# Wenlin-Chen/ADKF-IFT

Measured on AMD Instinct MI355X. Metric: meta-tasks/sec (N_support=128, d=256), higher is better.
Workload: dtype f32

## Files before the change

### adkf_ift_amd/csrc/adkf_gp.hip

```cpp
#include <hip/hip_runtime.h>
#include <algorithm>
#include <cstdio>
#include <cstdlib>

#include "../../include/adkf_gp.h"
#include "ard.h"
#include "pna.h"
#include "readout.h"
#include "block.h"
#include "outer_step.h"
#include "refine64.h"
#include "hyper.h"
#include "large_fused.h"
#include "gemm_x3.h"
#include "dense_x3.h"
#include "dist_task.h"
#include "dz_task.h"
#include "predict_stream.h"
#include "thompson_stream.h"
#include "believer_stream.h"
#include "mes_stream.h"
#include "gumbel_stream.h"
#include "gibbon_stream.h"
#include "kg_stream.h"
#include "jes_stream.h"
#include "ipv_stream.h"
#include "jackknife_stream.h"
#include "ehvi_stream.h"
#include "mix_stream.h"

#include "host_common.h"
#include "host_gp.h"
#include "host_ard.h"
#include "host_stream.h"

extern "C" {

const char* adkf_last_hip_error(void) { return hipGetErrorString(g_last_hip_error); }

const char* adkf_version(void) { return "adkf_gp 0.1 (gfx950)"; }

int adkf_path_info(int32_t ns_max, int32_t nq_max) {
    if (ns_max <= 0 || nq_max < 0 || ns_max > MAX_POINTS || nq_max > MAX_POINTS) return ADKF_E_SIZE;
    int bits = 0;
    const int hi = ns_max > nq_max ? ns_max : nq_max;
    if (nq_max > 0 && use_fused_outer(ns_max, nq_max)) bits |= ADKF_PATH_FUSED_OUTER;
    if (hi > REG_POINTS) { bits |= ADKF_PATH_BLOCKED; if (lg_fused_by_size(hi)) bits |= ADKF_PATH_BLOCKED_FUSED; }
    if (carve(nullptr, 1, ns_max, nq_max > 0 ? nq_max : 1, 4).w64_stride != 0) bits |= ADKF_PATH_R64_REGION;
    if (refine64_lds_optin()) bits |= ADKF_PATH_R64_LDS;
    return bits;
}

int adkf_max_points(void) { return MAX_POINTS; }

size_t adkf_workspace_bytes(int32_t T, int32_t ns_max, int32_t nq_max, int32_t d) {
    if (T <= 0 || ns_max <= 0 || nq_max < 0 || d <= 0) return 0;
    return carve(nullptr, T, ns_max, nq_max, d).bytes;
}

size_t adkf_workspace_bytes_ard(int32_t T, int32_t ns_max, int32_t nq_max, int32_t d) {
    if (T <= 0 || ns_max <= 0 || nq_max < 0 || d <= 0) return 0;
    return carve_ard(nullptr, carve(nullptr, T, ns_max, nq_max, d).bytes, T, ns_max, nq_max, d).bytes;
}

static int median_core(const adkf_batch_t* b, const Workspace& w, float* l0, const InitArgs& init, bool* fused, hipStream_t st) {
    int rc = stage_dist(b, w, has_query(b), st);
    if (rc) return rc;
    *fused = b->ns_max <= 256;
    if (b->ns_max <= 128) k_median<512, 16><<<grid_for(b->T, 1), 512, 0, st>>>(w.D2ss, b->n_s, b->ns_max, l0, b->T, init);
    else if (b->ns_max <= 256) k_median<1024, 32><<<grid_for(b->T, 1), 1024, 0, st>>>(w.D2ss, b->n_s, b->ns_max, l0, b->T, init);
    else {
        LgMedian lm{w.D2ss, b->n_s, b->ns_max, l0, b->T, reinterpret_cast<uint32_t*>(w.lg_med), w.lg_med + b->T, w.lg_med + 2 * (size_t)b->T};
        hipMemsetAsync(lm.hist, 0, sizeof(int) * 256 * (size_t)b->T, st);
        const int rows_blocks = ceil_div(b->ns_max, 16) < 64 ? ceil_div(b->ns_max, 16) : 64;
        for (int pass = 0; pass < 4; ++pass) {
            k_lg_med_hist<<<dim3(rows_blocks, b->T), 256, 0, st>>>(lm, pass);
            k_lg_med_pick<<<ceil_div(b->T, 64), 64, 0, st>>>(lm, pass);
        }
    }
    LAUNCH_OK();
    return 0;
}

int adkf_median_lengthscale(const adkf_batch_t* b, float* l0, void* ws, size_t ws_bytes, void* stream) {
    int rc = check_batch(b, false);
    if (rc) return rc;
    if (!l0 || !ws) return ADKF_E_BADARG;
    Workspace w = carve_for(b, ws);
    if (ws_bytes < w.bytes) return ADKF_E_WORKSPACE;
    bool fused;
    return median_core(b, w, l0, InitArgs{0, 0, nullptr, nullptr}, &fused, static_cast<hipStream_t>(stream));
}

int adkf_init_params(const adkf_batch_t* b, int32_t use_numeric_labels, int32_t use_lengthscale_prior, float* phi,
                     float* priors, float* l0, void* ws, size_t ws_bytes, void* stream) {
    int rc = check_batch(b, false);
    if (rc) return rc;
    if (!phi || !priors || !ws) return ADKF_E_BADARG;
    Workspace w = carve_for(b, ws);
    if (ws_bytes < w.bytes) return ADKF_E_WORKSPACE;
    float* l0p = l0 ? l0 : w.l0;
    hipStream_t st = static_cast<hipStream_t>(stream);
    InitArgs init{use_numeric_labels, use_lengthscale_prior, phi, priors};
    ArdWs a{};
    if (is_ard(b)) {
        a = carve_ard(ws, w.bytes, b->T, b->ns_max, b->nq_max, b->d);
        if (ws_bytes < a.bytes) return ADKF_E_WORKSPACE;
        init.phi = a.phi3;
    }
    bool fused = false;
    rc = median_core(b, w, l0p, init, &fused, st);
    if (rc) return rc;
    if (!fused) k_init_params<<<ceil_div(b->T, 64), 64, 0, st>>>(l0p, b->T, init);
    if (is_ard(b)) k_ard_expand_phi<<<dim3(ceil_div(2 + b->d, 256), b->T), 256, 0, st>>>(a.phi3, phi, b->T, 2 + b->d);
    LAUNCH_OK();
    return 0;
}

int adkf_mll_value_grad(const adkf_batch_t* b, const float* phi, float* f_in, float* g_phi, float* dZ_s, int32_t* info,
                        void* ws, size_t ws_bytes, void* stream) {
    int rc = check_batch(b, false);
    if (rc) return rc;
    if (!phi || !f_in || !info || !ws || !b->y_s || !b->priors) return ADKF_E_BADARG;
    if (is_ard(b)) {
        ArdCtx c;
        adkf_batch_t b0 = *b; b0.flags &= ~ADKF_BATCH_REUSE_INNER;
        rc = ard_setup(&b0, ws, ws_bytes, static_cast<hipStream_t>(stream), c);
        if (rc) return rc;
        rc = ard_eval(c, phi, f_in, g_phi ? g_phi : c.a.ge, info);
        if (rc) return rc;
        if (dZ_s) {
            ArdDzFin fs{c.v, c.a.G, nullptr, nullptr, nullptr, 0.f, dZ_s, b->n_s, c.ns};
            k_ard_dz_fin<<<dim3(ceil_div(c.d, 256), c.ns, c.T), 256, 0, c.st>>>(fs);
            LAUNCH_OK();
        }
        return 0;
    }
    Workspace w = carve_for(b, ws);
    if (ws_bytes < w.bytes) return ADKF_E_WORKSPACE;
    hipStream_t st = static_cast<hipStream_t>(stream);
    rc = stage_dist(b, w, has_query(b), st);
    if (rc) return rc;
    InnerArgs ia = inner_args(b, w, const_cast<float*>(phi), info);
    ia.f_out = f_in; ia.g_out = g_phi;
    rc = launch_inner(ia, w, st);
    if (rc) return rc;
    launch_refine(make_tv(b, w, false), b, w, false, 0, nullptr, info, st, f_in, g_phi, nullptr);
    if (dZ_s) {
        TaskView tv = make_tv(b, w, false);
        const int win_tiles = std::max(1, std::min(64, b->ns_max * b->ns_max / 2048));
        WinArgs wa{tv, w.Ainv, w.D2ss, w.Wss, w.scal, b->T, win_tiles};
// ... 295 lines not shown
```

### adkf_ift_amd/csrc/dist_task.h

```cpp
#pragma once
#include "kernels.h"
#include "gemm_x3.h"

namespace adkf {

constexpr int DT_N = 128, DT_NT = 512, DT_PLANE = DT_N * X3_RS, DT_OPER = 3 * DT_PLANE, DT_BUF = 2 * DT_OPER;
constexpr int DT_LDS_BYTES = 2 * DT_BUF * (int)sizeof(unsigned short);

struct DistTaskArgs {
    const float *Zs, *Zq, *mean;
    float *D2ss, *D2qs, *D2qq;
    int d, T;
};

extern __shared__ __attribute__((aligned(16))) unsigned short dt_lds[];

__global__ __launch_bounds__(DT_NT) void k_dist_task(DistTaskArgs a) {
    constexpr int MI = 4, MJ = 2, IH = 1;
    int t, tile;
    if (!task_tile(a.T, 1, t, tile)) return;
    __shared__ float rowsq[2][DT_N];
    const int tid = threadIdx.x, lane = tid & 63, wv = tid >> 6;
    const int wr = wv >> 2, wc = (wv & 3) ^ (wr << 1), fi = lane & 15, fk = lane >> 4;
    const int d = a.d, nc = d / GK, last = nc - 1;
    const bool sym_on = !(wr == 1 && wc < 2);

    const int sr = tid >> 3, sk = (tid & 7) * 4;
    const char* const zs = reinterpret_cast<const char*>(a.Zs + (size_t)t * DT_N * d);
    const char* const zq = reinterpret_cast<const char*>(a.Zq + (size_t)t * DT_N * d);
    const char* const mu = reinterpret_cast<const char*>(a.mean + (size_t)t * d);
    const size_t hi = (size_t)256 * d;
    const uint32_t off = 4u * (uint32_t)(sr * d + sk), off_mu = 4u * (uint32_t)sk;
    auto ldb = [](const char* base, uint32_t o) __attribute__((always_inline)) { return *reinterpret_cast<const float4*>(base + o); };
    const int frag_a = (wr * 64 + fi) * X3_RS + 8 * fk, frag_b = (wc * 32 + fi) * X3_RS + 8 * fk;

    float4 rs[2][2], rq[2][2], rm;
    float sqs[2] = {0.f, 0.f}, sqq[2] = {0.f, 0.f};
    auto fetch = [&](auto with_s, int set, int c) __attribute__((always_inline)) {
        const size_t k = (size_t)(4 * GK) * c;
        if constexpr (decltype(with_s)::value) { rs[set][0] = ldb(zs + k, off); rs[set][1] = ldb(zs + hi + k, off); }
        rq[set][0] = ldb(zq + k, off); rq[set][1] = ldb(zq + hi + k, off);
    };
    auto fetch_mean = [&](int c) __attribute__((always_inline)) { rm = ldb(mu + (size_t)(4 * GK) * c, off_mu); };
    auto centre = [](const float4& r, const float4& m, float (&v)[4]) __attribute__((always_inline)) {
        constexpr int DPP_IDENTITY = 0xE4;
        v[0] = dpp_f<DPP_IDENTITY>(r.x) - m.x; v[1] = dpp_f<DPP_IDENTITY>(r.y) - m.y;
        v[2] = dpp_f<DPP_IDENTITY>(r.z) - m.z; v[3] = dpp_f<DPP_IDENTITY>(r.w) - m.w;
    };
    auto stage = [&](auto with_s, int buf, int set, bool commit) __attribute__((always_inline)) {
        constexpr bool S = decltype(with_s)::value;
        unsigned short* B = dt_lds + buf * DT_BUF;
        float v[2][4], ts[2] = {sqs[0], sqs[1]}, tq[2] = {sqq[0], sqq[1]};
        if constexpr (S) {
            centre(rs[set][0], rm, v[0]); centre(rs[set][1], rm, v[1]);
            x3_stage<true, DT_N, DT_NT, 1>(B, v, ts);
        }
        centre(rq[set][0], rm, v[0]); centre(rq[set][1], rm, v[1]);
        x3_stage<true, DT_N, DT_NT, S ? 1 : 0>(B + DT_OPER, v, tq);
        if constexpr (S) {
#pragma unroll
            for (int ps = 0; ps < 2; ++ps) { sqs[ps] = commit ? ts[ps] : sqs[ps]; sqq[ps] = commit ? tq[ps] : sqq[ps]; }
        }
    };

    auto block_terms = [&](const unsigned short* Ab, const unsigned short* Bb, const bf16x8 (&b)[2][MJ], f32x4 (&acc)[MI][MJ], f32x4 (&small)[MI][MJ]) __attribute__((always_inline)) {
#define ADKF_DT_LOADA(dst_, q_) _Pragma("unroll") for (int i = 0; i < IH; ++i) dst_[i] = *reinterpret_cast<const bf16x8*>(Ab + (q_) * DT_PLANE + (ih + i) * 16 * X3_RS);
#define ADKF_DT_TERM(dst_, av_, bq_)                                                                       \
    _Pragma("unroll") for (int i = 0; i < IH; ++i) _Pragma("unroll") for (int j = 0; j < MJ; ++j)        \
        dst_[ih + i][j] = __builtin_amdgcn_mfma_f32_16x16x32_bf16(bq_[j], av_[i], dst_[ih + i][j], 0, 0, 0);
#pragma unroll
        for (int ih = 0; ih < MI; ih += IH) {
            bf16x8 a0[IH], ax[IH], b2[MJ];
#pragma unroll
            for (int j = 0; j < MJ; ++j) b2[j] = *reinterpret_cast<const bf16x8*>(Bb + 2 * DT_PLANE + j * 16 * X3_RS);
            ADKF_DT_LOADA(a0, 0) ADKF_DT_TERM(small, a0, b2)
            ADKF_DT_LOADA(ax, 2) ADKF_DT_TERM(small, ax, b[0])
            ADKF_DT_LOADA(ax, 1) ADKF_DT_TERM(small, ax, b[1])
            ADKF_DT_TERM(acc, a0, b[0])
            ADKF_DT_TERM(small, a0, b[1]) ADKF_DT_TERM(small, ax, b[0])
        }
#undef ADKF_DT_TERM
#undef ADKF_DT_LOADA
    };
    auto load_b = [&](const unsigned short* Bb, bf16x8 (&b)[2][MJ]) __attribute__((always_inline)) {
#pragma unroll
        for (int q = 0; q < 2; ++q)
#pragma unroll
            for (int j = 0; j < MJ; ++j) b[q][j] = *reinterpret_cast<const bf16x8*>(Bb + q * DT_PLANE + j * 16 * X3_RS);
    };
    auto run_pass = [&](auto with_s, auto&& multiply) __attribute__((always_inline)) {
        auto advance = [&](int c, int nbuf, int nset, bool commit) __attribute__((always_inline)) {
            stage(with_s, nbuf, nset, commit);
            fetch_mean(min(c + 2, last));
            __builtin_amdgcn_sched_barrier(0);
            fetch(with_s, nset, min(c + 3, last));
        };
        stage(with_s, 0, 0, true);
        fetch_mean(min(1, last));
        __builtin_amdgcn_sched_barrier(0);
        fetch(with_s, 0, min(2, last));
        __syncthreads();
        int c = 0;
        for (; c + 1 < nc; c += 2) {
            multiply(0); advance(c, 1, 1, true); __syncthreads();
            multiply(1); advance(c + 1, 0, 0, c + 2 < nc); __syncthreads();
        }
        if (c < nc) { multiply(0); __syncthreads(); }
    };
    auto zero = [](f32x4 (&x)[MI][MJ]) __attribute__((always_inline)) {
#pragma unroll
        for (int i = 0; i < MI; ++i)
#pragma unroll
            for (int j = 0; j < MJ; ++j) x[i][j] = (f32x4){0.f, 0.f, 0.f, 0.f};
    };
    auto values = [&](const f32x4& acc, const float* nrow, const float* ncol, int gi, int gj0, float (&v)[4]) __attribute__((always_inline)) {
        const float nx = nrow[gi];
        const float4 ny = *reinterpret_cast<const float4*>(ncol + gj0);
        v[0] = fmaxf(nx + ny.x - 2.f * acc[0], 0.f); v[1] = fmaxf(nx + ny.y - 2.f * acc[1], 0.f);
        v[2] = fmaxf(nx + ny.z - 2.f * acc[2], 0.f); v[3] = fmaxf(nx + ny.w - 2.f * acc[3], 0.f);
    };
    auto store_sym = [&](float* D, const f32x4& acc, const float* nrm, int rt, int ct) __attribute__((always_inline)) {
        const int gi = rt * 16 + fi, gj0 = ct * 16 + fk * 4;
        float v[4];
        values(acc, nrm, nrm, gi, gj0, v);
        if (rt < ct) {
            *reinterpret_cast<float4*>(D + (size_t)gi * DT_N + gj0) = make_float4(v[0], v[1], v[2], v[3]);
#pragma unroll
            for (int r = 0; r < 4; ++r) D[(size_t)(gj0 + r) * DT_N + gi] = v[r];
        } else {
#pragma unroll
            for (int r = 0; r < 4; ++r) {
                const int gj = gj0 + r;
                if (gi == gj) D[(size_t)gi * DT_N + gj] = 0.f;
                else if (gi < gj) { D[(size_t)gi * DT_N + gj] = v[r]; D[(size_t)gj * DT_N + gi] = v[r]; }
            }
        }
    };

    const std::true_type pass1{};
    const std::false_type pass2{};
    float* const Dss = a.D2ss + (size_t)t * DT_N * DT_N;
    float* const Dqs = a.D2qs + (size_t)t * DT_N * DT_N;
    float* const Dqq = a.D2qq + (size_t)t * DT_N * DT_N;

    fetch_mean(0);
    __builtin_amdgcn_sched_barrier(0);
    fetch(pass1, 0, 0); fetch(pass1, 1, min(1, last));
    {
        f32x4 acc_s[MI][MJ], small_s[MI][MJ], acc_q[MI][MJ], small_q[MI][MJ];
        zero(acc_s); zero(small_s); zero(acc_q); zero(small_q);
        run_pass(pass1, [&](int buf) __attribute__((always_inline)) {
            const unsigned short* S = dt_lds + buf * DT_BUF;
            bf16x8 b[2][MJ];
            load_b(S + frag_b, b);
            if (sym_on) block_terms(S + frag_a, S + frag_b, b, acc_s, small_s);
            __builtin_amdgcn_sched_barrier(0);
            block_terms(S + DT_OPER + frag_a, S + frag_b, b, acc_q, small_q);
        });
        fetch_mean(0);
        __builtin_amdgcn_sched_barrier(0);
        fetch(pass2, 0, 0); fetch(pass2, 1, min(1, last));
#pragma unroll
        for (int ps = 0; ps < 2; ++ps) {
            float s = sqs[ps], q = sqq[ps];
            s += dpp_f<DPP_XOR1>(s); s += dpp_f<DPP_XOR2>(s); s += dpp_f<DPP_HALF_MIRROR>(s);
            q += dpp_f<DPP_XOR1>(q); q += dpp_f<DPP_XOR2>(q); q += dpp_f<DPP_HALF_MIRROR>(q);
            if ((tid & 7) == 0) { rowsq[0][sr + ps * 64] = s; rowsq[1][sr + ps * 64] = q; }
        }
        __syncthreads();
#pragma unroll
        for (int i = 0; i < MI; ++i)
#pragma unroll
            for (int j = 0; j < MJ; ++j) {
                const int rt = wr * 4 + i, ct = wc * 2 + j;
                float v[4];
                values(acc_q[i][j] + small_q[i][j], rowsq[1], rowsq[0], rt * 16 + fi, ct * 16 + fk * 4, v);
                *reinterpret_cast<float4*>(Dqs + (size_t)(rt * 16 + fi) * DT_N + ct * 16 + fk * 4) = make_float4(v[0], v[1], v[2], v[3]);
                if (rt <= ct) store_sym(Dss, acc_s[i][j] + small_s[i][j], rowsq[0], rt, ct);
            }
    }

    {
        f32x4 acc_g[MI][MJ], small_g[MI][MJ];
        zero(acc_g); zero(small_g);
        run_pass(pass2, [&](int buf) __attribute__((always_inline)) {
            if (sym_on) {
                const unsigned short* Q = dt_lds + buf * DT_BUF + DT_OPER;
                bf16x8 b[2][MJ];
                load_b(Q + frag_b, b);
                block_terms(Q + frag_a, Q + frag_b, b, acc_g, small_g);
            }
        });
#pragma unroll
        for (int i = 0; i < MI; ++i)
#pragma unroll
            for (int j = 0; j < MJ; ++j) {
                const int rt = wr * 4 + i, ct = wc * 2 + j;
                if (rt <= ct) store_sym(Dqq, acc_g[i][j] + small_g[i][j], rowsq[1], rt, ct);
            }
    }
}

}
```

### adkf_ift_amd/csrc/host_gp.h

```cpp
#pragma once
#include "host_common.h"

namespace {

inline bool x3_for(int d) { return d >= GK; }

struct Workspace {
    float *mean, *D2ss, *D2qs, *D2qq, *Ainv, *P, *C, *S, *OC, *Wss, *Wqs, *Wqq, *vecs, *scal, *part_oc, *part_ma, *l0;
    float *lg_Dinv, *lg_C, *lg_F, *lg_logdet, *lg_part, *lg_pext;
    int32_t *lg_info, *lg_med, *lg_cnt;
    FitShared* lg_fit;
    double* w64; size_t w64_stride;
    int vld, nt_oc, nt_ma;
    int lg_mode;
    size_t bytes;
};

Workspace carve(void* base, int T, int ns, int nq, int d) {
    Workspace w{};
    Arena ar{static_cast<char*>(base), 0};
    const size_t Tz = (size_t)T;
    w.vld = ns > nq ? ns : nq;
    w.nt_oc = nq > 0 ? tiles_of(nq, ns) : 0;
    w.nt_ma = tiles_of(ns, ns);
    w.mean = ar.floats(Tz * d);
    w.D2ss = ar.floats(Tz * ns * ns);
    w.D2qs = ar.floats(Tz * nq * ns);
    w.D2qq = ar.floats(Tz * nq * nq);
    w.Ainv = ar.floats(Tz * ns * ns);
    w.P = ar.floats(Tz * ns * ns);
    w.C = ar.floats(Tz * nq * ns);
    w.S = ar.floats(Tz * nq * nq);
    w.OC = ar.floats(Tz * nq * ns);
    w.Wss = ar.floats(Tz * ns * ns);
    w.Wqs = ar.floats(Tz * nq * ns);
    w.Wqq = ar.floats(Tz * nq * nq);
    w.vecs = ar.floats(Tz * NVEC * w.vld);
    w.scal = ar.floats(Tz * NSCAL);
    w.part_oc = ar.floats(Tz * (w.nt_oc > 0 ? w.nt_oc : 1) * 4);
    w.part_ma = ar.floats(Tz * w.nt_ma * 4);
    w.l0 = ar.floats(Tz);
    if (w.vld > REG_POINTS) {
        w.lg_Dinv = ar.floats(2 * Tz * LB * LB);
        w.lg_C = ar.floats(Tz * LB * w.vld);
        w.lg_F = ar.floats(Tz * LB * w.vld);
        w.lg_logdet = ar.floats(Tz);
        w.lg_pext = ar.floats(Tz * 2);
        const size_t tq = (size_t)((nq + GT - 1) / GT) * ((nq + GT - 1) / GT);
        const size_t ts = (size_t)((ns + GT - 1) / GT) * ((ns + GT - 1) / GT);
        w.lg_part = ar.floats(Tz * (ts > tq ? ts : tq) * 8);
        w.lg_info = ar.as<int32_t>(Tz);
        w.lg_cnt = ar.as<int32_t>(Tz);
        w.lg_med = ar.as<int32_t>(Tz * 258);
        static_assert(sizeof(FitShared) % sizeof(float) == 0, "FitShared is carved as whole floats");
        w.lg_fit = ar.as<FitShared>(Tz);
    }
    if (w.vld <= r64_maxn()) {
        w.w64_stride = refine64_doubles(ns, nq);
        w.w64 = ar.as<double>(Tz * w.w64_stride);
    }
    w.bytes = ar.off;
    return w;
}

Workspace carve_for(const adkf_batch_t* b, void* ws) {
    Workspace w = carve(ws, b->T, b->ns_max, b->nq_max, b->d);
    w.lg_mode = (b->flags & ADKF_BATCH_LG_UNFUSED) ? -1 : (b->flags & ADKF_BATCH_LG_FUSED) ? 1 : 0;
    return w;
}

int check_batch(const adkf_batch_t* b, bool need_query) {
    (void)hipGetLastError();
    if (!b || b->T <= 0 || b->ns_max <= 0 || b->d <= 0 || !b->Z_s) return ADKF_E_BADARG;
    if (b->kernel != ADKF_KERNEL_RBF && b->kernel != ADKF_KERNEL_MATERN52) return ADKF_E_BADARG;
    if (b->ns_max > MAX_POINTS) return ADKF_E_SIZE;
    if (need_query) {
        if (b->nq_max <= 0 || !b->Z_q) return ADKF_E_BADARG;
        if (b->nq_max > MAX_POINTS) return ADKF_E_SIZE;
    }
    return 0;
}

bool vec_ok(const adkf_batch_t* b, const Workspace& w) {
    if ((b->ns_max & 3) || (b->nq_max & 3) || (b->d & 3) || (w.vld & 3)) return false;
    return aligned16(b->Z_s) && aligned16(b->Z_q) && aligned16(w.mean);
}

TaskView make_tv(const adkf_batch_t* b, const Workspace& w, bool with_query) {
    TaskView tv;
    tv.n_s = b->n_s; tv.n_q = with_query ? b->n_q : nullptr;
    tv.ns_ld = b->ns_max; tv.nq_ld = with_query ? b->nq_max : 0; tv.vld = w.vld; tv.kind = b->kernel;
    tv.scal = w.scal; tv.vecs = w.vecs;
    tv.vec = vec_ok(b, w);
    return tv;
}

inline bool has_query(const adkf_batch_t* b) { return b->nq_max > 0 && b->Z_q != nullptr; }
inline bool is_ard(const adkf_batch_t* b) { return (b->flags & ADKF_BATCH_ARD) != 0; }

bool use_dist_task(const adkf_batch_t* b, const Workspace& w, bool with_query, int parts) {
    static const bool optin = lds_optin(DT_LDS_BYTES, {kernel_ptr(&k_dist_task)});
    return optin && parts == 3 && with_query && b->ns_max == DT_N && b->nq_max == DT_N && !b->n_s && !b->n_q && (b->d % GK) == 0 &&
           b->d <= (1 << 22) && vec_ok(b, w);
}

int stage_dist(const adkf_batch_t* b, const Workspace& w, bool with_query, hipStream_t st, int parts = 3) {
    if (b->flags & ADKF_BATCH_REUSE_DIST) return 0;
    const int T = b->T, ns = b->ns_max, nq = with_query ? b->nq_max : 0, d = b->d;
    if (!(parts & 2)) with_query = false;
    if ((parts & 1) && !(parts & 4)) k_colmean<<<dim3(ceil_div(d, 64), T), 256, 0, st>>>(b->Z_s, b->n_s, ns, d, w.mean, T);
    if (use_dist_task(b, w, with_query, parts)) {
        k_dist_task<<<grid_for(T, 1), DT_NT, DT_LDS_BYTES, st>>>(DistTaskArgs{b->Z_s, b->Z_q, w.mean, w.D2ss, w.D2qs, w.D2qq, d, T});
        LAUNCH_OK();
        return 0;
    }
    ProbDist p;
    p.mean = w.mean; p.d = d; p.vec = vec_ok(b, w);
    ProbDistMulti pm;
    pm.vec = p.vec; pm.end0 = pm.end1 = 0; pm.tn0 = pm.tn1 = pm.tn2 = 1;
    int nblk = 0, total = 0;
    auto add = [&](const ProbDist& q, int M, int N) {
        const int tn = ceil_div(N, GT), tiles = ceil_div(M, GT) * tn;
        if (nblk == 0) { pm.s0 = q; pm.tn0 = tn; pm.end0 = pm.end1 = total + tiles; pm.s1 = pm.s2 = q; }
        else if (nblk == 1) { pm.s1 = q; pm.tn1 = tn; pm.end1 = total + tiles; pm.s2 = q; }
        else { pm.s2 = q; pm.tn2 = tn; }
        total += tiles; ++nblk;
    };
    if (parts & 1) {
        p.X = b->Z_s; p.Y = b->Z_s; p.n_x = b->n_s; p.n_y = b->n_s; p.x_ld = ns; p.y_ld = ns; p.symmetric = true; p.D2 = w.D2ss;
        add(p, ns, ns);
    }
    if (with_query) {
        p.X = b->Z_q; p.Y = b->Z_s; p.n_x = b->n_q; p.n_y = b->n_s; p.x_ld = nq; p.y_ld = ns; p.symmetric = false; p.D2 = w.D2qs;
        add(p, nq, ns);
        p.X = b->Z_q; p.Y = b->Z_q; p.n_x = b->n_q; p.n_y = b->n_q; p.x_ld = nq; p.y_ld = nq; p.symmetric = true; p.D2 = w.D2qq;
        add(p, nq, nq);
    }
    if (nblk > 0) {
        if (x3_for(d)) k_bgemm3<ProbDistMulti, GT, 256><<<grid_for(T, total), 256, 0, st>>>(pm, T, 1, total);
        else k_bgemm<ProbDistMulti, GT><<<grid_for(T, total), 256, 0, st>>>(pm, T, 1, total);
    }
    LAUNCH_OK();
    return 0;
}

template <int NMAX, int NT, bool LOW>
void launch_inner_kl(const InnerArgs& a, hipStream_t st) {
    constexpr size_t cache_bytes = sizeof(float) * NMAX * NMAX;
    static const bool optin = lds_optin(cache_bytes, {kernel_ptr(&k_inner<NMAX, NT, 0, LOW>), kernel_ptr(&k_inner<NMAX, NT, 1, LOW>)});
    (void)optin;
    if (a.kind == ADKF_KERNEL_RBF) k_inner<NMAX, NT, 0, LOW><<<grid_for(a.T, 1), NT, cache_bytes, st>>>(a);
    else k_inner<NMAX, NT, 1, LOW><<<grid_for(a.T, 1), NT, cache_bytes, st>>>(a);
}

template <int NMAX, int NT>
void launch_inner_k(const InnerArgs& a, hipStream_t st) {
    if constexpr (NMAX == 128) {
        if (a.T > num_cus()) { launch_inner_kl<NMAX, NT, true>(a, st); return; }
    }
    launch_inner_kl<NMAX, NT, false>(a, st);
}

inline bool lg_fused_by_size(int ld) { return ld >= 4 * LB; }

LgMat lg_mat(const Workspace& w, float* M, int ld, const int32_t* n_arr, const FitShared* fit, int T) {
    LgMat m;
    m.M = M; m.ld = ld; m.n_arr = n_arr; m.fit = fit;
    m.Dinv = w.lg_Dinv; m.Cbuf = w.lg_C; m.Fbuf = w.lg_F; m.logdet = w.lg_logdet; m.pext = w.lg_pext; m.info = w.lg_info;
    const bool fused = w.lg_mode > 0 || (w.lg_mode == 0 && lg_fused_by_size(ld));
    m.cnt = fused ? w.lg_cnt : nullptr;
    m.T = T; m.vec = (ld & 3) == 0;
    return m;
}

void lg_sweep(const LgMat& m0, hipStream_t st) {
    const int nb = ceil_div(m0.ld, LB), tn = ceil_div(m0.ld, GT);
    LgMat m = m0;
    if (m.cnt) {
        float* dinv[2] = {m0.Dinv, m0.Dinv + (size_t)m0.T * LB * LB};
        const int npair = lgf_npair(tn);
        k_lg_diag<<<grid_for(m.T, 1), 512, 0, st>>>(m, 0);
        for (int step = 0; step < nb; ++step) {
            m.Dinv = dinv[step & 1];
            ProbLgPanel pp; pp.m = m; pp.step = step;
            k_bgemm<ProbLgPanel><<<grid_for(m.T, 2 * tn), 256, 0, st>>>(pp, m.T, 2, tn);
            LgStepArgs sa{m, dinv[(step + 1) & 1], m.cnt, step, tn, npair, step + 1 < nb ? 1 : 0};
            k_lg_update_sweep<<<grid_for(m.T, npair), LGF_NT, 0, st>>>(sa);
        }
        return;
    }
    for (int step = 0; step < nb; ++step) {
        k_lg_diag<<<grid_for(m.T, 1), 512, 0, st>>>(m, step);
        ProbLgPanel pp; pp.m = m; pp.step = step;
        k_bgemm<ProbLgPanel><<<grid_for(m.T, 2 * tn), 256, 0, st>>>(pp, m.T, 2, tn);
        ProbLgUpdate pu; pu.m = m; pu.step = step; pu.tri = tn * (tn + 1) / 2;
        k_bgemm<ProbLgUpdate><<<grid_for(m.T, pu.tri), 256, 0, st>>>(pu, m.T, tn, tn);
// ... 265 lines not shown
```

### adkf_ift_amd/csrc/kernels.h

```cpp
#pragma once
#include "problems.h"
#include "inner.h"

namespace adkf {

__global__ __launch_bounds__(256) void k_colmean(const float* Zs, const int32_t* n_s, int ns_ld, int d, float* mean, int T) {
    __shared__ float part[16][64];
    const int t = blockIdx.y;
    const int n = n_s ? n_s[t] : ns_ld;
    const float* Z = Zs + (size_t)t * ns_ld * d;
    const bool vec = (d & 3) == 0 && (reinterpret_cast<uintptr_t>(Zs) & 15) == 0;
    if (vec) {
        const int q = threadIdx.x & 15, g = threadIdx.x >> 4, c4 = blockIdx.x * 64 + q * 4;
        float4 s = make_float4(0.f, 0.f, 0.f, 0.f);
        if (c4 < d) {
            for (int i0 = g; i0 < n; i0 += 16 * 8) {
                float4 v[8];
#pragma unroll
                for (int u = 0; u < 8; ++u) {
                    const int i = i0 + 16 * u;
                    v[u] = *reinterpret_cast<const float4*>(Z + (size_t)(i < n ? i : n - 1) * d + c4);
                }
#pragma unroll
                for (int u = 0; u < 8; ++u)
                    if (i0 + 16 * u < n) { s.x += v[u].x; s.y += v[u].y; s.z += v[u].z; s.w += v[u].w; }
            }
        }
        *reinterpret_cast<float4*>(&part[g][q * 4]) = s;
        __syncthreads();
        const int cl = threadIdx.x, c = blockIdx.x * 64 + cl;
        if (cl < 64 && c < d) {
            float r = 0.f;
#pragma unroll
            for (int k = 0; k < 16; ++k) r += part[k][cl];
            mean[(size_t)t * d + c] = n > 0 ? r / (float)n : 0.f;
        }
        return;
    }
    const int cl = threadIdx.x & 63, g = threadIdx.x >> 6;
    const int c = blockIdx.x * 64 + cl;
    float s = 0.f;
    if (c < d)
        for (int i = g; i < n; i += 4) s += Z[(size_t)i * d + c];
    part[g][cl] = s;
    __syncthreads();
    if (g == 0 && c < d) {
        s = (part[0][cl] + part[1][cl]) + (part[2][cl] + part[3][cl]);
        mean[(size_t)t * d + c] = n > 0 ? s / (float)n : 0.f;
    }
}

struct ProbDist {
    static constexpr bool A_KCONTIG = true, B_KCONTIG = true;
    static constexpr int NRED = 0;
    const float *X, *Y, *mean; const int32_t *n_x, *n_y; int x_ld, y_ld, d; bool symmetric; float* D2;
    int mx, my, i_base, j_base; const float *Xi, *Yi, *mu, *nxi, *nyi; float* Do; bool vec;
    __device__ bool setup(int t) {
        mx = n_x ? n_x[t] : x_ld; my = n_y ? n_y[t] : y_ld;
        Xi = X + (size_t)t * x_ld * d; Yi = Y + (size_t)t * y_ld * d; mu = mean + (size_t)t * d;
        nxi = nyi = nullptr; Do = D2 + (size_t)t * x_ld * y_ld;
        return mx > 0 && my > 0;
    }
    __device__ int M() const { return mx; } __device__ int N() const { return my; } __device__ int K() const { return d; }
    __device__ float a(int i, int k) const { return Xi[(size_t)i * d + k] - mu[k]; }
    __device__ float b(int k, int j) const { return Yi[(size_t)j * d + k] - mu[k]; }
    static constexpr int A_NRAW = 2, B_NRAW = 2;
    __device__ bool raw_ok() const { return true; }
    __device__ void a_raw(int i, int k, float4 (&r)[2]) const { r[0] = ldq(Xi + (size_t)i * d + k); r[1] = ldq(mu + k); }
    __device__ void b_raw(int k, int j, float4 (&r)[2]) const { r[0] = ldq(Yi + (size_t)j * d + k); r[1] = ldq(mu + k); }
    __device__ void a_fin(int, int, const float4 (&r)[2], float (&v)[4]) const {
        v[0] = r[0].x - r[1].x; v[1] = r[0].y - r[1].y; v[2] = r[0].z - r[1].z; v[3] = r[0].w - r[1].w;
    }
    __device__ void b_fin(int k, int j, const float4 (&r)[2], float (&v)[4]) const { a_fin(j, k, r, v); }
    __device__ void a4(int i, int k, float (&v)[4]) const { float4 r[2]; a_raw(i, k, r); a_fin(i, k, r, v); }
    __device__ void b4(int k, int j, float (&v)[4]) const { float4 r[2]; b_raw(k, j, r); b_fin(k, j, r, v); }
    __device__ bool active(int m0, int n0) const { return !symmetric || m0 <= n0; }
    __device__ void set_rowsq(const float* a, const float* b, int m0, int n0) { nxi = a; nyi = b; i_base = m0; j_base = n0; }
    __device__ float value(int i, int j, float acc) const {
        const float v = fmaxf(nxi[i - i_base] + nyi[j - j_base] - 2.f * acc, 0.f);
        return (symmetric && i == j) ? 0.f : v;
    }
    __device__ void epi(int i, int j, float acc, float*) const {
        if (symmetric && i > j) return;
        const float v = value(i, j, acc);
        Do[(size_t)i * y_ld + j] = v;
        if (symmetric && i < j) Do[(size_t)j * y_ld + i] = v;
    }
    __device__ void epi4(int i0, int j, const float (&acc)[4], float* red) const {
        if (!(symmetric && vec && i0 + 3 < j)) {
#pragma unroll
            for (int r = 0; r < 4; ++r) epi(i0 + r, j, acc[r], red);
            return;
        }
        float v[4];
#pragma unroll
        for (int r = 0; r < 4; ++r) { v[r] = value(i0 + r, j, acc[r]); Do[(size_t)(i0 + r) * y_ld + j] = v[r]; }
        *reinterpret_cast<float4*>(Do + (size_t)j * y_ld + i0) = make_float4(v[0], v[1], v[2], v[3]);
    }
    __device__ void store_red(int, const float*) const {}
};

struct ProbDistMulti {
    static constexpr bool A_KCONTIG = true, B_KCONTIG = true;
    static constexpr int NRED = 0;
    ProbDist s0, s1, s2; int end0, end1, tn0, tn1, tn2;
    ProbDist q; bool vec;
    __device__ void select(int& tile, int& tiles_n) {
        if (tile < end0) { q = s0; tiles_n = tn0; }
        else if (tile < end1) { q = s1; tiles_n = tn1; tile -= end0; }
        else { q = s2; tiles_n = tn2; tile -= end1; }
    }
    __device__ bool setup(int t) { return q.setup(t); }
    __device__ int M() const { return q.M(); } __device__ int N() const { return q.N(); } __device__ int K() const { return q.K(); }
    __device__ float a(int i, int k) const { return q.a(i, k); }
    __device__ float b(int k, int j) const { return q.b(k, j); }
    __device__ void a4(int i, int k, float (&v)[4]) const { q.a4(i, k, v); }
    __device__ void b4(int k, int j, float (&v)[4]) const { q.b4(k, j, v); }
    static constexpr int A_NRAW = 2, B_NRAW = 2;
    __device__ bool raw_ok() const { return true; }
    __device__ void a_raw(int i, int k, float4 (&r)[2]) const { q.a_raw(i, k, r); }
    __device__ void b_raw(int k, int j, float4 (&r)[2]) const { q.b_raw(k, j, r); }
    __device__ void a_fin(int i, int k, const float4 (&r)[2], float (&v)[4]) const { q.a_fin(i, k, r, v); }
    __device__ void b_fin(int k, int j, const float4 (&r)[2], float (&v)[4]) const { q.b_fin(k, j, r, v); }
    __device__ bool active(int m0, int n0) const { return q.active(m0, n0); }
    __device__ void epi(int i, int j, float acc, float* red) const { q.epi(i, j, acc, red); }
    __device__ void epi4(int i0, int j, const float (&acc)[4], float* red) const { q.epi4(i0, j, acc, red); }
    __device__ void set_rowsq(const float* a, const float* b, int m0, int n0) { q.set_rowsq(a, b, m0, n0); }
    __device__ void store_red(int, const float*) const {}
};

struct InitArgs { int numeric, use_ls_prior; float* phi; float* priors; };

__device__ __forceinline__ void init_params_task(const InitArgs& a, int t, float l0) {
    const float scale = 0.25f;
    const float mode = a.numeric ? 0.01f : 0.1f;
    a.phi[t * 3 + 0] = inv_softplus_f(mode - NOISE_LB);
    a.phi[t * 3 + 1] = 0.f;
    a.phi[t * 3 + 2] = inv_softplus_f(l0);
    a.priors[t * 4 + 0] = logf(mode) + scale * scale;
    a.priors[t * 4 + 1] = scale;
    a.priors[t * 4 + 2] = a.use_ls_prior ? logf(l0) + scale * scale : 0.f;
    a.priors[t * 4 + 3] = a.use_ls_prior ? scale : -1.f;
}

__global__ void k_init_params(const float* l0, int T, InitArgs a) {
    const int t = blockIdx.x * blockDim.x + threadIdx.x;
    if (t < T) init_params_task(a, t, l0[t]);
}

template <int NT, int EPT>
__global__ __launch_bounds__(NT) void k_median(const float* D2ss, const int32_t* n_s, int ld, float* l0, int T, InitArgs init) {
    constexpr int NW = NT / 64;
    __shared__ int red[2][NW];
    int t, tile;
    if (!task_tile(T, 1, t, tile)) return;
    const int n = n_s ? n_s[t] : ld;
    const uint32_t* D = reinterpret_cast<const uint32_t*>(D2ss + (size_t)t * ld * ld);
    const int tid = threadIdx.x, lane = tid & 63, wv = tid >> 6;
    if (n <= 1 || n > ld) {
        if (tid == 0) { l0[t] = 0.f; if (init.phi) init_params_task(init, t, 0.f); }
        return;
    }
    const int nm1 = n - 1, slots = ((n + 1) >> 1) * nm1;
    uint32_t v[EPT];
    int nonzero = 0;
#pragma unroll
    for (int r = 0; r < EPT; ++r) {
        const int e = r * NT + tid;
        const int ec = e < slots ? e : slots - 1;
        const int fr = ec / nm1, c = ec - fr * nm1, top = nm1 - fr;
        const int i = c < top ? fr : top, j = c < top ? fr + 1 + c : top + 1 + (c - top);
        uint32_t val = D[(size_t)i * ld + j];
        if (!(e < slots && (c < top || top != fr))) val = 0u;
        v[r] = val;
        nonzero += __popcll(__ballot(val != 0u));
    }
    const int zeros = EPT * 64 - nonzero;
    if (lane == 0) red[0][wv] = nonzero;
    __syncthreads();
    int total = 0;
#pragma unroll
    for (int i = 0; i < NW; ++i) total += red[0][i];
    if (total == 0) { if (tid == 0) { l0[t] = 0.f; if (init.phi) init_params_task(init, t, 0.f); } return; }
    int rank = (total - 1) / 2;
    uint32_t prefix = 0;
    int buf = 1;
    for (int bit = 30; bit >= 0; --bit, buf ^= 1) {
        const uint32_t hi_mask = ~((1u << bit) - 1u);
        int c0 = 0;
#pragma unroll
        for (int r = 0; r < EPT; ++r) c0 += __popcll(__ballot((v[r] & hi_mask) == prefix));
        if (prefix == 0u) c0 -= zeros;
        if (lane == 0) red[buf][wv] = c0;
        __syncthreads();
        c0 = 0;
#pragma unroll
        for (int i = 0; i < NW; ++i) c0 += red[buf][i];
        if (rank >= c0) { rank -= c0; prefix |= (1u << bit); }
    }
    if (tid == 0) {
        const float l = sqrtf(0.5f * __uint_as_float(prefix));
        l0[t] = l;
        if (init.phi) init_params_task(init, t, l);
    }
}

struct HessArgs { TaskView tv; const float* Ainv; const float* P; const float* D2ss; const float* y_s; const float* priors; float* scal; float* vecs; int T; };

constexpr int SMALL_NT = 1024;

__device__ __forceinline__ void hess_assemble(float* sc, const float* pri, int n, const float* acc) {
    const float noise = sc[S_NOISE], os = sc[S_OS], ls = sc[S_LS];
    const float trA2 = acc[0], trPA = acc[1], trPP = acc[2], trAinvKll = acc[3], aKlla = acc[4], ag = acc[5], bg = acc[6], bd = acc[7], ab = acc[8];
    const float trAinv = sc[S_TRAINV], aa = sc[S_AA], ya = sc[S_YA], trAinvG = sc[S_TRAINVG], aGa = sc[S_AGA];
    const float fn = (float)n;
    float h00 = ag - 0.5f * trA2;
    const float h01 = ((aa - noise * ag) - 0.5f * (trAinv - noise * trA2)) / os;
    const float h02 = bg - 0.5f * trPA;
    const float h11 = ((ya - 2.f * noise * aa + noise * noise * ag) - 0.5f * (fn - 2.f * noise * trAinv + noise * noise * trA2)) / (os * os);
    const float h12 = ((ab - noise * bg) - 0.5f * (trAinvG - noise * trPA)) / os - (0.5f * aGa - 0.5f * trAinvG) / os;
    float h22 = bd - 0.5f * aKlla - 0.5f * trPP + 0.5f * trAinvKll;
    if (pri[1] > 0.f) { const float lx = logf(noise), s2 = pri[1] * pri[1]; h00 -= (1.f + (lx - pri[0]) / s2 - 1.f / s2) / (noise * noise); }
    if (pri[3] > 0.f) { const float lx = logf(ls), s2 = pri[3] * pri[3]; h22 -= (1.f + (lx - pri[2]) / s2 - 1.f / s2) / (ls * ls); }
    const float d1[3] = {sc[S_D1N], sc[S_D1S], sc[S_D1L]}, d2[3] = {sc[S_D2N], sc[S_D2S], sc[S_D2L]};
    const float gt[3] = {sc[S_GT0], sc[S_GT1], sc[S_GT2]};
    const float h[3][3] = {{h00, h01, h02}, {h01, h11, h12}, {h02, h12, h22}};
    for (int i = 0; i < 3; ++i)
        for (int j = 0; j < 3; ++j) sc[S_H0 + i * 3 + j] = (h[i][j] * d1[i] * d1[j] + (i == j ? gt[i] * d2[i] : 0.f)) / fn;
}

__global__ __launch_bounds__(SMALL_NT) void k_hess(HessArgs a) {
    constexpr int NT = SMALL_NT, NW = NT / 64;
    __shared__ float red[9 * NW];
    int t, tile;
    if (!task_tile(a.T, 1, t, tile)) return;
    const int n = a.tv.ns(t), ld = a.tv.ns_ld, tid = threadIdx.x, lane = tid & 63, wv = tid >> 6;
    float* sc = a.scal + (size_t)t * NSCAL;
    const float os = sc[S_OS], ls = sc[S_LS], il2 = 1.f / (ls * ls);
    const float* Ai = a.Ainv + (size_t)t * ld * ld;
    const float* Pi = a.P + (size_t)t * ld * ld;
    const float* D2 = a.D2ss + (size_t)t * ld * ld;
    float* al = a.vecs + ((size_t)t * NVEC + V_ALPHA) * a.tv.vld;
    float* be = a.vecs + ((size_t)t * NVEC + V_BETA) * a.tv.vld;
    float* ga = a.vecs + ((size_t)t * NVEC + V_GAMMA) * a.tv.vld;
    float* de = a.vecs + ((size_t)t * NVEC + V_DELTA) * a.tv.vld;
    const int kind = a.tv.kind;
    constexpr int RF = 8;
    for (int i0 = wv; i0 < n; i0 += RF * NW) {
        float sb[RF], sg[RF];
#pragma unroll
        for (int q = 0; q < RF; ++q) { sb[q] = 0.f; sg[q] = 0.f; }
        for (int j = lane; j < n; j += 64) {
            const float aj = al[j];
            float d2v[RF], av[RF];
#pragma unroll
            for (int q = 0; q < RF; ++q) {
                const int i = i0 + q * NW, ic = i < n ? i : n - 1;
                d2v[q] = D2[(size_t)ic * ld + j];
                av[q] = Ai[(size_t)ic * ld + j];
            }
#pragma unroll
            for (int q = 0; q < RF; ++q) {
                float k0, k1, k2; const float u = d2v[q] * il2; kappa3(kind, u, k0, k1, k2);
                const bool in = i0 + q * NW < n;
                sb[q] += in ? os * k1 * u * (-2.f / ls) * aj : 0.f;
                sg[q] += in ? av[q] * aj : 0.f;
            }
        }
#pragma unroll
        for (int q = 0; q < RF; ++q) {
            const int i = i0 + q * NW;
            const float b_ = wave_sum(sb[q]), g_ = wave_sum(sg[q]);
            if (lane == 0 && i < n) { be[i] = b_; ga[i] = g_; }
        }
    }
    __threadfence_block();
    __syncthreads();
    for (int i0 = wv; i0 < n; i0 += RF * NW) {
        float sd[RF];
#pragma unroll
        for (int q = 0; q < RF; ++q) sd[q] = 0.f;
        for (int j = lane; j < n; j += 64) {
            const float bj = be[j];
            float av[RF];
#pragma unroll
            for (int q = 0; q < RF; ++q) { const int i = i0 + q * NW; av[q] = Ai[(size_t)(i < n ? i : n - 1) * ld + j]; }
#pragma unroll
// ... 358 lines not shown
```

Measured before the change: 306,000.

## Fuse median lengthscale selection into distance kernel with radix-histogram select

The median of the pairwise support distances is now computed inside the per-task distance kernel from register-resident values, so the separate median kernel and its reload of D2ss are skipped when the fused distance path is used. The 31-step bitwise radix select is replaced by a shared histogram select that takes 11-bit digits and first narrows the range with a min/max reduction, which cuts the number of block-wide barriers. The trade is more registers and LDS work in the distance kernel's epilogue, plus LDS atomics for the histogram.

```diff
diff --git a/adkf_ift_amd/csrc/adkf_gp.hip b/adkf_ift_amd/csrc/adkf_gp.hip
--- a/adkf_ift_amd/csrc/adkf_gp.hip
+++ b/adkf_ift_amd/csrc/adkf_gp.hip
@@ -64,9 +64,11 @@
 }
 
 static int median_core(const adkf_batch_t* b, const Workspace& w, float* l0, const InitArgs& init, bool* fused, hipStream_t st) {
-    int rc = stage_dist(b, w, has_query(b), st);
+    bool selected = false;
+    int rc = stage_dist(b, w, has_query(b), st, 3, l0, &init, &selected);
     if (rc) return rc;
     *fused = b->ns_max <= 256;
+    if (selected) return 0;
     if (b->ns_max <= 128) k_median<512, 16><<<grid_for(b->T, 1), 512, 0, st>>>(w.D2ss, b->n_s, b->ns_max, l0, b->T, init);
     else if (b->ns_max <= 256) k_median<1024, 32><<<grid_for(b->T, 1), 1024, 0, st>>>(w.D2ss, b->n_s, b->ns_max, l0, b->T, init);
     else {
diff --git a/adkf_ift_amd/csrc/dist_task.h b/adkf_ift_amd/csrc/dist_task.h
--- a/adkf_ift_amd/csrc/dist_task.h
+++ b/adkf_ift_amd/csrc/dist_task.h
@@ -11,10 +11,15 @@
     const float *Zs, *Zq, *mean;
     float *D2ss, *D2qs, *D2qq;
     int d, T;
+    float* l0;
+    InitArgs init;
 };
 
+static_assert(MedianSelect<MEDIAN_W>::WORDS * (int)sizeof(uint32_t) <= DT_LDS_BYTES, "the select's histograms live in the staging buffers");
+
 extern __shared__ __attribute__((aligned(16))) unsigned short dt_lds[];
 
+template <bool SELECT>
 __global__ __launch_bounds__(DT_NT) void k_dist_task(DistTaskArgs a) {
     constexpr int MI = 4, MJ = 2, IH = 1;
     int t, tile;
@@ -119,9 +124,8 @@
         v[0] = fmaxf(nx + ny.x - 2.f * acc[0], 0.f); v[1] = fmaxf(nx + ny.y - 2.f * acc[1], 0.f);
         v[2] = fmaxf(nx + ny.z - 2.f * acc[2], 0.f); v[3] = fmaxf(nx + ny.w - 2.f * acc[3], 0.f);
     };
-    auto store_sym = [&](float* D, const f32x4& acc, const float* nrm, int rt, int ct) __attribute__((always_inline)) {
+    auto store_sym = [&](float* D, const f32x4& acc, const float* nrm, int rt, int ct, float (&v)[4]) __attribute__((always_inline)) {
         const int gi = rt * 16 + fi, gj0 = ct * 16 + fk * 4;
-        float v[4];
         values(acc, nrm, nrm, gi, gj0, v);
         if (rt < ct) {
             *reinterpret_cast<float4*>(D + (size_t)gi * DT_N + gj0) = make_float4(v[0], v[1], v[2], v[3]);
@@ -168,6 +172,7 @@
             if ((tid & 7) == 0) { rowsq[0][sr + ps * 64] = s; rowsq[1][sr + ps * 64] = q; }
         }
         __syncthreads();
+        uint32_t key[SELECT ? MI * MJ * 4 : 1];
 #pragma unroll
         for (int i = 0; i < MI; ++i)
 #pragma unroll
@@ -176,8 +181,18 @@
                 float v[4];
                 values(acc_q[i][j] + small_q[i][j], rowsq[1], rowsq[0], rt * 16 + fi, ct * 16 + fk * 4, v);
                 *reinterpret_cast<float4*>(Dqs + (size_t)(rt * 16 + fi) * DT_N + ct * 16 + fk * 4) = make_float4(v[0], v[1], v[2], v[3]);
-                if (rt <= ct) store_sym(Dss, acc_s[i][j] + small_s[i][j], rowsq[0], rt, ct);
-            }
+                if (rt <= ct) store_sym(Dss, acc_s[i][j] + small_s[i][j], rowsq[0], rt, ct, v);
+                if constexpr (SELECT) {
+#pragma unroll
+                    for (int r = 0; r < 4; ++r)
+                        key[(i * MJ + j) * 4 + r] = (rt <= ct && rt * 16 + fi < ct * 16 + fk * 4 + r) ? __float_as_uint(v[r]) : 0u;
+                }
+            }
+        if constexpr (SELECT) {
+            const uint32_t bits = median_select<DT_NT, MI * MJ * 4, MEDIAN_W>(key, reinterpret_cast<uint32_t*>(dt_lds));
+            __syncthreads();
+            if (tid == 0) median_finish(a.init, t, a.l0, bits);
+        }
     }
 
     {
@@ -196,7 +211,8 @@
 #pragma unroll
             for (int j = 0; j < MJ; ++j) {
                 const int rt = wr * 4 + i, ct = wc * 2 + j;
-                if (rt <= ct) store_sym(Dqq, acc_g[i][j] + small_g[i][j], rowsq[1], rt, ct);
+                float v[4];
+                if (rt <= ct) store_sym(Dqq, acc_g[i][j] + small_g[i][j], rowsq[1], rt, ct, v);
             }
     }
 }
diff --git a/adkf_ift_amd/csrc/host_gp.h b/adkf_ift_amd/csrc/host_gp.h
--- a/adkf_ift_amd/csrc/host_gp.h
+++ b/adkf_ift_amd/csrc/host_gp.h
@@ -99,19 +99,24 @@
 inline bool is_ard(const adkf_batch_t* b) { return (b->flags & ADKF_BATCH_ARD) != 0; }
 
 bool use_dist_task(const adkf_batch_t* b, const Workspace& w, bool with_query, int parts) {
-    static const bool optin = lds_optin(DT_LDS_BYTES, {kernel_ptr(&k_dist_task)});
+    static const bool optin = lds_optin(DT_LDS_BYTES, {kernel_ptr(&k_dist_task<false>), kernel_ptr(&k_dist_task<true>)});
     return optin && parts == 3 && with_query && b->ns_max == DT_N && b->nq_max == DT_N && !b->n_s && !b->n_q && (b->d % GK) == 0 &&
            b->d <= (1 << 22) && vec_ok(b, w);
 }
 
-int stage_dist(const adkf_batch_t* b, const Workspace& w, bool with_query, hipStream_t st, int parts = 3) {
+int stage_dist(const adkf_batch_t* b, const Workspace& w, bool with_query, hipStream_t st, int parts = 3, float* l0 = nullptr,
+               const InitArgs* init = nullptr, bool* selected = nullptr) {
+    if (selected) *selected = false;
     if (b->flags & ADKF_BATCH_REUSE_DIST) return 0;
     const int T = b->T, ns = b->ns_max, nq = with_query ? b->nq_max : 0, d = b->d;
     if (!(parts & 2)) with_query = false;
     if ((parts & 1) && !(parts & 4)) k_colmean<<<dim3(ceil_div(d, 64), T), 256, 0, st>>>(b->Z_s, b->n_s, ns, d, w.mean, T);
     if (use_dist_task(b, w, with_query, parts)) {
-        k_dist_task<<<grid_for(T, 1), DT_NT, DT_LDS_BYTES, st>>>(DistTaskArgs{b->Z_s, b->Z_q, w.mean, w.D2ss, w.D2qs, w.D2qq, d, T});
+        const DistTaskArgs a{b->Z_s, b->Z_q, w.mean, w.D2ss, w.D2qs, w.D2qq, d, T, l0, init ? *init : InitArgs{0, 0, nullptr, nullptr}};
+        if (l0 && selected) k_dist_task<true><<<grid_for(T, 1), DT_NT, DT_LDS_BYTES, st>>>(a);
+        else k_dist_task<false><<<grid_for(T, 1), DT_NT, DT_LDS_BYTES, st>>>(a);
         LAUNCH_OK();
+        if (l0 && selected) *selected = true;
         return 0;
     }
     ProbDist p;
diff --git a/adkf_ift_amd/csrc/kernels.h b/adkf_ift_amd/csrc/kernels.h
--- a/adkf_ift_amd/csrc/kernels.h
+++ b/adkf_ift_amd/csrc/kernels.h
@@ -1,6 +1,7 @@
 #pragma once
 #include "problems.h"
 #include "inner.h"
+#include "median_select.h"
 
 namespace adkf {
 
@@ -148,22 +149,28 @@
     if (t < T) init_params_task(a, t, l0[t]);
 }
 
+constexpr int MEDIAN_W = 11;
+
+__device__ __forceinline__ void median_finish(const InitArgs& init, int t, float* l0, uint32_t bits) {
+    const float l = sqrtf(0.5f * __uint_as_float(bits));
+    l0[t] = l;
+    if (init.phi) init_params_task(init, t, l);
+}
+
 template <int NT, int EPT>
 __global__ __launch_bounds__(NT) void k_median(const float* D2ss, const int32_t* n_s, int ld, float* l0, int T, InitArgs init) {
-    constexpr int NW = NT / 64;
-    __shared__ int red[2][NW];
+    __shared__ __attribute__((aligned(16))) uint32_t sel[MedianSelect<MEDIAN_W>::WORDS];
     int t, tile;
     if (!task_tile(T, 1, t, tile)) return;
     const int n = n_s ? n_s[t] : ld;
     const uint32_t* D = reinterpret_cast<const uint32_t*>(D2ss + (size_t)t * ld * ld);
-    const int tid = threadIdx.x, lane = tid & 63, wv = tid >> 6;
+    const int tid = threadIdx.x;
     if (n <= 1 || n > ld) {
-        if (tid == 0) { l0[t] = 0.f; if (init.phi) init_params_task(init, t, 0.f); }
+        if (tid == 0) median_finish(init, t, l0, 0u);
         return;
     }
     const int nm1 = n - 1, slots = ((n + 1) >> 1) * nm1;
     uint32_t v[EPT];
-    int nonzero = 0;
 #pragma unroll
     for (int r = 0; r < EPT; ++r) {
         const int e = r * NT + tid;
@@ -173,36 +180,9 @@
         uint32_t val = D[(size_t)i * ld + j];
         if (!(e < slots && (c < top || top != fr))) val = 0u;
         v[r] = val;
-        nonzero += __popcll(__ballot(val != 0u));
-    }
-    const int zeros = EPT * 64 - nonzero;
-    if (lane == 0) red[0][wv] = nonzero;
-    __syncthreads();
-    int total = 0;
-#pragma unroll
-    for (int i = 0; i < NW; ++i) total += red[0][i];
-    if (total == 0) { if (tid == 0) { l0[t] = 0.f; if (init.phi) init_params_task(init, t, 0.f); } return; }
-    int rank = (total - 1) / 2;
-    uint32_t prefix = 0;
-    int buf = 1;
-    for (int bit = 30; bit >= 0; --bit, buf ^= 1) {
-        const uint32_t hi_mask = ~((1u << bit) - 1u);
-        int c0 = 0;
-#pragma unroll
-        for (int r = 0; r < EPT; ++r) c0 += __popcll(__ballot((v[r] & hi_mask) == prefix));
-        if (prefix == 0u) c0 -= zeros;
-        if (lane == 0) red[buf][wv] = c0;
-        __syncthreads();
-        c0 = 0;
-#pragma unroll
-        for (int i = 0; i < NW; ++i) c0 += red[buf][i];
-        if (rank >= c0) { rank -= c0; prefix |= (1u << bit); }
-    }
-    if (tid == 0) {
-        const float l = sqrtf(0.5f * __uint_as_float(prefix));
-        l0[t] = l;
-        if (init.phi) init_params_task(init, t, l);
-    }
+    }
+    const uint32_t bits = median_select<NT, EPT, MEDIAN_W>(v, sel);
+    if (tid == 0) median_finish(init, t, l0, bits);
 }
 
 struct HessArgs { TaskView tv; const float* Ainv; const float* P; const float* D2ss; const float* y_s; const float* priors; float* scal; float* vecs; int T; };
diff --git a/adkf_ift_amd/csrc/median_select.h b/adkf_ift_amd/csrc/median_select.h
--- /dev/null
+++ b/adkf_ift_amd/csrc/median_select.h
@@ -0,0 +1,112 @@
+#pragma once
+#include "device_utils.h"
+
+namespace adkf {
+
+template <int W>
+struct MedianSelect {
+    static_assert(W >= 7 && W <= 13, "2^W bins, at least two per lane of a scanning wave");
+    static constexpr int NB = 1 << W, BPL = NB / 64;
+    static constexpr int HIST = NB + 64;
+    static constexpr int PASSES = (31 + W - 1) / W;
+    static constexpr int HEAD = 64 * 4;
+    static constexpr int WORDS = HEAD + PASSES * HIST;
+    __device__ static constexpr int slot(int b) { return b + b / BPL; }
+};
+
+__device__ __forceinline__ int wave_scan_i(int v) {
+    constexpr int ROW_SHR = 0x110;
+    v += dpp_i<ROW_SHR + 1>(v);
+    v += dpp_i<ROW_SHR + 2>(v);
+    v += dpp_i<ROW_SHR + 4>(v);
+    v += dpp_i<ROW_SHR + 8>(v);
+    const int t0 = __builtin_amdgcn_readlane(v, 15), t1 = __builtin_amdgcn_readlane(v, 31), t2 = __builtin_amdgcn_readlane(v, 47);
+    const int row = (threadIdx.x & 63) >> 4;
+    return v + (row >= 1 ? t0 : 0) + (row >= 2 ? t1 : 0) + (row >= 3 ? t2 : 0);
+}
+__device__ __forceinline__ uint32_t wave_umin(uint32_t v) {
+    v = min(v, (uint32_t)dpp_i<DPP_XOR1>((int)v)); v = min(v, (uint32_t)dpp_i<DPP_XOR2>((int)v));
+    v = min(v, (uint32_t)dpp_i<DPP_HALF_MIRROR>((int)v)); v = min(v, (uint32_t)dpp_i<DPP_MIRROR>((int)v));
+    const int b = (int)v;
+    return min(min((uint32_t)__builtin_amdgcn_readlane(b, 0), (uint32_t)__builtin_amdgcn_readlane(b, 16)),
+               min((uint32_t)__builtin_amdgcn_readlane(b, 32), (uint32_t)__builtin_amdgcn_readlane(b, 48)));
+}
+__device__ __forceinline__ uint32_t wave_umax(uint32_t v) { return ~wave_umin(~v); }
+
+template <int NT, int K, int W>
+__device__ __forceinline__ uint32_t median_select(const uint32_t (&key)[K], uint32_t* lds) {
+    using M = MedianSelect<W>;
+    constexpr int NW = NT / 64;
+    static_assert(NW <= 16 && NT % 64 == 0, "the header has room for sixteen waves");
+    const int tid = threadIdx.x, lane = tid & 63, wv = tid >> 6;
+    uint32_t* const hist = lds + M::HEAD;
+
+    int count = 0;
+    uint32_t lo = 0xFFFFFFFFu, hi = 0u;
+#pragma unroll
+    for (int r = 0; r < K; ++r) {
+        count += __popcll(__ballot(key[r] != 0u));
+        lo = min(lo, key[r] != 0u ? key[r] : 0xFFFFFFFFu);
+        hi = max(hi, key[r]);
+    }
+    lo = wave_umin(lo); hi = wave_umax(hi);
+    if (lane == 0) { lds[4 * wv] = (uint32_t)count; lds[4 * wv + 1] = lo; lds[4 * wv + 2] = hi; }
+    for (int i = tid * 4; i < M::PASSES * M::HIST; i += NT * 4) *reinterpret_cast<uint4*>(hist + i) = make_uint4(0u, 0u, 0u, 0u);
+    __syncthreads();
+    int total = 0;
+    lo = 0xFFFFFFFFu; hi = 0u;
+#pragma unroll
+    for (int i = 0; i < NW; ++i) {
+        const uint4 h = *reinterpret_cast<const uint4*>(lds + 4 * i);
+        total += (int)h.x; lo = min(lo, h.y); hi = max(hi, h.z);
+    }
+    if (total == 0) return 0u;
+    if (lo == hi) return lo;
+    int rank = (total - 1) / 2;
+    int nb = min(32 - __clz((int)(lo ^ hi)), 31);
+    uint32_t prefix = (lo >> nb) << nb;
+
+    for (int p = 0; nb > 0; ++p) {
+        const int w = min(W, nb), shift = nb - w;
+        const uint32_t dmask = (1u << w) - 1u;
+        uint32_t* const h = hist + p * M::HIST;
+#pragma unroll
+        for (int r = 0; r < K; ++r) {
+            const bool live = key[r] != 0u && (key[r] >> nb) == (prefix >> nb);
+            const unsigned long long act = __ballot(live);
+            if (act == 0ull) continue;
+            const int dg = (int)((key[r] >> shift) & dmask);
+            const int first = __ffsll(act) - 1;
+            const int d0 = __builtin_amdgcn_readlane(dg, first);
+            const unsigned long long same = __ballot(live && dg == d0);
+            if (lane == first) atomicAdd(h + M::slot(d0), (uint32_t)__popcll(same));
+            else if (live && dg != d0) atomicAdd(h + M::slot(dg), 1u);
+        }
+        __syncthreads();
+        int c[M::BPL], s = 0;
+#pragma unroll
+        for (int j = 0; j < M::BPL; ++j) c[j] = (int)h[lane * (M::BPL + 1) + j];
+        __builtin_amdgcn_sched_barrier(0);
+#pragma unroll
+        for (int j = 0; j < M::BPL; ++j) s += c[j];
+        const int incl = wave_scan_i(s), excl = incl - s;
+        const int local = rank - excl;
+        int below = 0, bin = 0, cum = 0;
+#pragma unroll
+        for (int j = 0; j < M::BPL; ++j) {
+            cum += c[j];
+            const bool under = cum <= local;
+            bin += under ? 1 : 0;
+            below = under ? cum : below;
+        }
+        const unsigned long long own = __ballot(local >= 0 && local < s);
+        const int o = __ffsll(own) - 1;
+        const int digit = __builtin_amdgcn_readlane(lane * M::BPL + bin, o);
+        rank = __builtin_amdgcn_readlane(local - below, o);
+        prefix |= ((uint32_t)digit & dmask) << shift;
+        nb = shift;
+    }
+    return prefix;
+}
+
+}
```

After: 309,200 (median of 6 runs). 1.01x the previous value.
